# KingOfTheAce2/video-restoration-pipeline-framewright

Measured on AMD Instinct MI355X. Metric: frames/sec Real-ESRGAN x4 1080p (RRDBNet-x4plus, 1920x1080 -> 7680x4320), higher is better.
Workload: dtype f16; 1 GPU; RealESRGAN_x4plus x4, 1920x1080 uint8 BGR frames resident in HBM -> 7680x4320 uint8 BGR in HBM, seeded synthetic weights, 43 frames per GPU

## Files before the change

video-restoration-pipeline-framewright_amd/csrc/conv3x3_wino.hip:

```cpp
#include <cstdlib>
#include <cstring>
#include <type_traits>
#include "fw_internal.h"
#include "conv_common.h"

namespace fw {

constexpr int WN_ROWP = 2 * 17 * 4;
constexpr int WN_ACT = HALO_H * WN_ROWP;
constexpr int WN_ACT_REGION = ACT_INSTR * 64;
constexpr int WN_WFR = 3 * 4 * 4;
constexpr int WN_W_REGION = WN_WFR * 64;
constexpr int WN_TOTAL = WN_ACT_REGION + 2 * WN_W_REGION;
static_assert(NWAVES == 8 && RPW == 2 && WN_TOTAL * 16 <= 160 * 1024, "written for 8 waves of 2 rows");

typedef _Float16 wn_h2 __attribute__((ext_vector_type(2)));
__device__ __forceinline__ uint4 wn_sub(uint4 a, uint4 b) {
    uint4 r;
    r.x = __builtin_bit_cast(unsigned, __builtin_bit_cast(wn_h2, a.x) - __builtin_bit_cast(wn_h2, b.x));
    r.y = __builtin_bit_cast(unsigned, __builtin_bit_cast(wn_h2, a.y) - __builtin_bit_cast(wn_h2, b.y));
    r.z = __builtin_bit_cast(unsigned, __builtin_bit_cast(wn_h2, a.z) - __builtin_bit_cast(wn_h2, b.z));
    r.w = __builtin_bit_cast(unsigned, __builtin_bit_cast(wn_h2, a.w) - __builtin_bit_cast(wn_h2, b.w));
    return r;
}
__device__ __forceinline__ uint4 wn_add(uint4 a, uint4 b) {
    uint4 r;
    r.x = __builtin_bit_cast(unsigned, __builtin_bit_cast(wn_h2, a.x) + __builtin_bit_cast(wn_h2, b.x));
    r.y = __builtin_bit_cast(unsigned, __builtin_bit_cast(wn_h2, a.y) + __builtin_bit_cast(wn_h2, b.y));
    r.z = __builtin_bit_cast(unsigned, __builtin_bit_cast(wn_h2, a.z) + __builtin_bit_cast(wn_h2, b.z));
    r.w = __builtin_bit_cast(unsigned, __builtin_bit_cast(wn_h2, a.w) + __builtin_bit_cast(wn_h2, b.w));
    return r;
}

__device__ __forceinline__ void wn_glds_w6(const void* sbase, unsigned voff, unsigned lds_piece4) {
    const unsigned long long b = (unsigned long long)sbase;
    const unsigned long long sb = ((unsigned long long)(unsigned)__builtin_amdgcn_readfirstlane((unsigned)(b >> 32)) << 32) |
                                  (unsigned long long)(unsigned)__builtin_amdgcn_readfirstlane((unsigned)b);
    lds_piece4 = __builtin_amdgcn_readfirstlane(lds_piece4);
    asm volatile(
        "s_nop 4\n\t"
        "s_mov_b32 m0, %2\n\t"
        "s_nop 0\n\t"
        "global_load_lds_dwordx4 %0, %1 offset:-4096\n\t"
        "global_load_lds_dwordx4 %0, %1 offset:-3072\n\t"
        "global_load_lds_dwordx4 %0, %1 offset:-2048\n\t"
        "global_load_lds_dwordx4 %0, %1 offset:-1024\n\t"
        "global_load_lds_dwordx4 %0, %1\n\t"
        "global_load_lds_dwordx4 %0, %1 offset:1024"
        :
        : "v"(voff), "s"(sb), "s"(lds_piece4)
        : "memory");
}

template <bool PLANES, bool STORE>
__global__ __launch_bounds__(64 * NWAVES, WAVES_PER_SIMD) void conv3x3_wino_split_kernel(const ConvParams p) {
    using T = _Float16;
    __shared__ __attribute__((aligned(16))) uint4 lds[WN_TOTAL];
    const int tid = threadIdx.x;
    const int wave = __builtin_amdgcn_readfirstlane(tid >> 6);
    const int lane = tid & 63;
    const int j = lane & 15;
    const int sl = lane >> 4;

    const int NB = gridDim.x;
    const int xcd = blockIdx.x & 7;
    const int qn = NB >> 3, rn = NB & 7;
    const int lb = (xcd < rn ? xcd * (qn + 1) : rn * (qn + 1) + (xcd - rn) * qn) + (blockIdx.x >> 3);
    const int tiles_x = (p.W + TILE_W - 1) / TILE_W;
    const int tiles_y = (p.H + TILE_H - 1) / TILE_H;
    const int ntiles = tiles_x * tiles_y;
    const int t_lo = (int)((long)lb * ntiles / NB);
    const int t_hi = (int)((long)(lb + 1) * ntiles / NB);
    if (t_lo >= t_hi) return;
    const int nch = p.cin_chunks;
    const int nitems = (t_hi - t_lo) * nch;

    unsigned relb[ACT_ITERS];
    auto piece_pos = [&](int i, int* row, int* px, int* s) {
        int idx = (ACT_ITERS * wave + i) * 64 + lane;
        if (idx >= WN_ACT) idx -= WN_ACT;
        const int rw = idx / WN_ROWP;
        const int rm = idx - rw * WN_ROWP;
        const int par = rm >= 68 ? 1 : 0;
        const int q = rm - 68 * par;
        const int ci = q >> 2;
        *row = rw;
        *px = 2 * ci + par;
        *s = (q & 3) ^ halo_swz(ci);
    };
#pragma unroll
    for (int i = 0; i < ACT_ITERS; ++i) {
        int row, px, s;
        piece_pos(i, &row, &px, &s);
        relb[i] = (unsigned)(((row * p.W + px) * p.in_cstride + s * 8) * 2) + (unsigned)(4 - i) * 1024u;
    }
    const unsigned lds_base = (unsigned)(size_t)(lds_ptr_t)lds;
    const char* in = reinterpret_cast<const char*>(p.in);
    const char* w_b = reinterpret_cast<const char*>(p.wpk);
    const unsigned lane16 = lane * 16;
    const long chunk_bytes = p.in_pstride * 2;

    unsigned a_ok = 0;
    bool a_all = true;
    const char* a_src = nullptr;
    int a_t = t_lo, a_c = 0;
    auto plan_tile = [&]() {
        int aty, atx;
        tile_pos(a_t, tiles_x, tiles_y, &aty, &atx);
        const int ty0 = aty * TILE_H, tx0 = atx * TILE_W;
        a_src = in + ((long)(ty0 - 1) * p.W + (tx0 - 1)) * p.in_cstride * 2;
        a_ok = 0;
#pragma unroll
        for (int i = 0; i < ACT_ITERS; ++i) {
            int row, px, s;
            piece_pos(i, &row, &px, &s);
            const int gy = ty0 - 1 + row, gx = tx0 - 1 + px;
            if ((unsigned)gy < (unsigned)p.H && (unsigned)gx < (unsigned)p.W) a_ok |= 1u << i;
        }
        a_all = __builtin_amdgcn_readfirstlane(__all(a_ok == (1u << ACT_ITERS) - 1u)) != 0;
    };
    auto issue_act = [&]() {
        if (a_c == 0) plan_tile();
        const unsigned dst = (unsigned)(ACT_ITERS * wave * 64);
        if (a_all) {
            glds16_batch_a(a_src, relb, lds_base + (dst + 4 * 64) * 16u);
        } else {
#pragma unroll
            for (int i = 0; i < ACT_ITERS; ++i)
                glds16_v(((a_ok >> i) & 1u) ? a_src + (relb[i] - (unsigned)(4 - i) * 1024u) : reinterpret_cast<const char*>(p.zeros),
                         lds_base + (dst + i * 64) * 16u);
        }
        if (++a_c == nch) {
            a_c = 0;
            ++a_t;
        } else {
            a_src += chunk_bytes;
        }
    };
    auto issue_w = [&](int c, int ws) {
        wn_glds_w6(w_b + (size_t)c * (WN_WFR * 1024) + (6 * wave + 4) * 1024, lane16,
                   lds_base + (unsigned)(WN_ACT_REGION + ws * WN_W_REGION + (6 * wave + 4) * 64) * 16u);
    };

    int rd[4];
#pragma unroll
    for (int k = 0; k < 4; ++k) {
        const int ci = j + (k >> 1);
        rd[k] = (k & 1) * 68 + ci * 4 + (sl ^ halo_swz(ci));
    }
    unsigned id_mask = 0;
#pragma unroll
    for (int ctl = 0; ctl < 2; ++ctl)
#pragma unroll
        for (int e = 0; e < 8; ++e)
            if (16 * ctl + j == 8 * sl + e) id_mask |= 1u << (8 * ctl + e);

    f32x4 acc[RPW][4][4];

    auto add_identity = [&](const uint4 (&xf)[RPW], float sc, int c2, auto freq_tag) {
        constexpr int F = decltype(freq_tag)::value;
#pragma unroll
        for (int ctl = 0; ctl < 2; ++ctl) {
            asm volatile("" : "+v"(sc));
            float e[8];
#pragma unroll
            for (int k = 0; k < 8; ++k) e[k] = ((id_mask >> (8 * ctl + k)) & 1u) ? sc : 0.f;
            const uint2 lo4 = Op<T>::pack4(e[0], e[1], e[2], e[3]);
            const uint2 hi4 = Op<T>::pack4(e[4], e[5], e[6], e[7]);
            const uint4 idf = make_uint4(lo4.x, lo4.y, hi4.x, hi4.y);
#pragma unroll
            for (int row = 0; row < RPW; ++row) {
                if (c2)
                    acc[row][F][2 + ctl] = Op<T>::mfma16(idf, xf[row], acc[row][F][2 + ctl]);
                else
                    acc[row][F][ctl] = Op<T>::mfma16(idf, xf[row], acc[row][F][ctl]);
            }
        }
    };

    auto add_identity1 = [&](int row, const uint4& xf, float sc, int c2, auto freq_tag) {
        constexpr int F = decltype(freq_tag)::value;
#pragma unroll
        for (int ctl = 0; ctl < 2; ++ctl) {
            asm volatile("" : "+v"(sc));
            float e[8];
#pragma unroll
            for (int k = 0; k < 8; ++k) e[k] = ((id_mask >> (8 * ctl + k)) & 1u) ? sc : 0.f;
            const uint2 lo4 = Op<T>::pack4(e[0], e[1], e[2], e[3]);
            const uint2 hi4 = Op<T>::pack4(e[4], e[5], e[6], e[7]);
            const uint4 idf = make_uint4(lo4.x, lo4.y, hi4.x, hi4.y);
            if (c2)
                acc[row][F][2 + ctl] = Op<T>::mfma16(idf, xf, acc[row][F][2 + ctl]);
            else
                acc[row][F][ctl] = Op<T>::mfma16(idf, xf, acc[row][F][ctl]);
        }
    };

    issue_w(0, 0);
    issue_act();

    int n = 0;
    for (int t = t_lo; t < t_hi; ++t) {
        int tty, ttx;
        tile_pos(t, tiles_x, tiles_y, &tty, &ttx);
        const int y0 = tty * TILE_H;
        const int x0 = ttx * TILE_W;
#pragma unroll
        for (int ct = 0; ct < 4; ++ct) {
            const f32x4 bv = *reinterpret_cast<const f32x4*>(p.bias + 16 * ct + 4 * sl);
#pragma unroll
            for (int row = 0; row < RPW; ++row) {
                acc[row][0][ct] = f32x4{0.f, 0.f, 0.f, 0.f};
                acc[row][1][ct] = bv;
                acc[row][2][ct] = f32x4{0.f, 0.f, 0.f, 0.f};
                acc[row][3][ct] = f32x4{0.f, 0.f, 0.f, 0.f};
            }
        }

        for (int c = 0; c < nch; ++c, ++n) {
            if (c > 0 || t == t_lo) FW_WAIT_VMCNT(0);
            __syncthreads();
            uint4 V[4][4];
            const bool own = !STORE && c < 2 && p.in_id_scale != 0.f;
#pragma unroll
            for (int r = 0; r < 4; ++r) {
                const uint4* row = lds + (RPW * wave + r) * WN_ROWP;
                const uint4 d0 = row[rd[0]], d1 = row[rd[1]], d2 = row[rd[2]], d3 = row[rd[3]];
                V[r][0] = wn_sub(d0, d2);
                V[r][1] = wn_add(d1, d2);
                V[r][2] = wn_sub(d2, d1);
                V[r][3] = wn_sub(d1, d3);
                if ((r == 1 || r == 2) && own) {
                    add_identity1(r - 1, d1, p.in_id_scale, c, std::integral_constant<int, 0>{});
                    add_identity1(r - 1, d2, -p.in_id_scale, c, std::integral_constant<int, 3>{});
                }
            }
            __syncthreads();
            const bool more = n + 1 < nitems;
            const int c1 = (c + 1 == nch) ? 0 : c + 1;
#ifndef FW_WN_DMA_K
#define FW_WN_DMA_K -1
#endif
            if (FW_WN_DMA_K < 0 && more) {
                issue_w(c1, (n + 1) & 1);
                issue_act();
            }
            uint4 ix0[RPW], ix1[RPW];
            const bool has_id = PLANES && c < p.n_id;
            const uint4* wl = lds + WN_ACT_REGION + (n & 1) * WN_W_REGION + lane;
#ifndef FW_WN_RING
#define FW_WN_RING 3
#endif
#ifndef FW_WN_RES_K
#define FW_WN_RES_K 17
#endif
            constexpr int RING = FW_WN_RING;
            uint4 wf[RING];
#pragma unroll
            for (int k = 0; k < RING - 1; ++k) wf[k] = wl[k * 64];
            FW_SB();
#pragma unroll
            for (int k = 0; k < WN_WFR; ++k) {
                const int dy = k / 16, f = (k / 4) & 3, ct = k & 3;
                if (k + RING - 1 < WN_WFR) wf[(k + RING - 1) % RING] = wl[(k + RING - 1) * 64];
                FW_SB();
                acc[0][f][ct] = Op<T>::mfma16(wf[k % RING], V[dy][f], acc[0][f][ct]);
                acc[1][f][ct] = Op<T>::mfma16(wf[k % RING], V[dy + 1][f], acc[1][f][ct]);
                FW_SB();
                if (k == FW_WN_DMA_K && more) {
                    issue_w(c1, (n + 1) & 1);
                    issue_act();
                    FW_SB();
                }
                if constexpr (PLANES) {
                    if (k == FW_WN_RES_K) {
                        const char* plane = reinterpret_cast<const char*>(p.in) + p.chunk_off[has_id ? c : 0];
#pragma unroll
                        for (int row = 0; row < RPW; ++row) {
                            const int y = y0 + RPW * wave + row, x = x0 + 2 * j;
                            const int cy = y < p.H ? y : p.H - 1, cx0 = x < p.W ? x : p.W - 1, cx1 = x + 1 < p.W ? x + 1 : p.W - 1;
                            const unsigned rowb = (unsigned)cy * (unsigned)p.W;
                            ix0[row] = *reinterpret_cast<const uint4*>(plane + ((rowb + cx0) * (unsigned)p.in_cstride + 8 * sl) * 2u);
                            ix1[row] = *reinterpret_cast<const uint4*>(plane + ((rowb + cx1) * (unsigned)p.in_cstride + 8 * sl) * 2u);
                        }
                        FW_SB();
                    }
                }
            }
            if constexpr (PLANES) {
                if (has_id) {
#pragma unroll
                    for (int row = 0; row < RPW; ++row) {
                        const int y = y0 + RPW * wave + row, x = x0 + 2 * j;
                        if (!(y < p.H && x < p.W)) ix0[row] = make_uint4(0, 0, 0, 0);
                        if (!(y < p.H && x + 1 < p.W)) ix1[row] = make_uint4(0, 0, 0, 0);
                    }
                    add_identity(ix0, p.id_scale[c], c & 1, std::integral_constant<int, 0>{});
                    add_identity(ix1, -p.id_scale[c], c & 1, std::integral_constant<int, 3>{});
                }
            }
        }

        FW_WAIT_VMCNT(0);
        const int ls = (sl & 1) ? 2 + (sl >> 1) : (sl >> 1);
        const int npass = (!STORE && p.out_lo) ? 2 : 1;
#pragma unroll
        for (int row = 0; row < RPW; ++row) {
            const int y = y0 + RPW * wave + row;
            if (y >= p.H) continue;
#pragma unroll
            for (int ct = 0; ct < 4; ++ct) {
                f32x4 ya = acc[row][0][ct] + acc[row][1][ct] + acc[row][2][ct];
                f32x4 yb = acc[row][1][ct] - acc[row][2][ct] - acc[row][3][ct];
                if constexpr (STORE) {
                    if (p.act == 1) {
                        ya = lrelu4(ya);
                        yb = lrelu4(yb);
                    }
                } else {
                    ya = ya * p.s1;
                    yb = yb * p.s1;
                }
                acc[row][0][ct] = ya;
                acc[row][3][ct] = yb;
            }
            for (int pass = 0; pass < npass; ++pass) {
                char* lane_base = reinterpret_cast<char*>(pass ? p.out_lo : p.out) + ((long)(2 * j) * p.out_cstride + p.out_coff + ls * 8) * 2;
                const long rowoff = ((long)y * p.W + x0) * p.out_cstride * 2;
#pragma unroll
                for (int e = 0; e < 2; ++e)
#pragma unroll
                    for (int c2 = 0; c2 < 2; ++c2) {
                        f32x4 oa = e ? acc[row][3][2 * c2] : acc[row][0][2 * c2], ob = e ? acc[row][3][2 * c2 + 1] : acc[row][0][2 * c2 + 1];
                        if (pass) {
                            oa = oa - Op<T>::unpack4(Op<T>::pack4(oa[0], oa[1], oa[2], oa[3]));
                            ob = ob - Op<T>::unpack4(Op<T>::pack4(ob[0], ob[1], ob[2], ob[3]));
                        }
                        const uint2 pa = Op<T>::pack4(oa[0], oa[1], oa[2], oa[3]);
                        const uint2 pb = Op<T>::pack4(ob[0], ob[1], ob[2], ob[3]);
                        const u32x2 sx = __builtin_amdgcn_permlane16_swap(pa.x, pb.x, false, false);
                        const u32x2 sy = __builtin_amdgcn_permlane16_swap(pa.y, pb.y, false, false);
                        if (x0 + 2 * j + e < p.W)
                            store16(lane_base + rowoff + (long)e * p.out_cstride * 2 + (long)c2 * p.out_pstride * 2, make_uint4(sx[0], sy[0], sx[1], sy[1]));
                    }
            }
        }
    }
}

#undef FW_SB

size_t pack_conv3x3_wino_weights(DType dt, const float* w, int cout, int cin, int cin_chunks, uint16_t* dst) {
    const size_t n = (size_t)cin_chunks * WN_WFR * 64 * 8;
    if (!dst) return n;
    size_t o = 0;
    for (int c = 0; c < cin_chunks; ++c)
        for (int dy = 0; dy < 3; ++dy)
            for (int f = 0; f < 4; ++f)
                for (int ct = 0; ct < 4; ++ct)
                    for (int lane = 0; lane < 64; ++lane)
                        for (int e = 0; e < 8; ++e) {
                            const int co = 16 * ct + (lane & 15), ci = 32 * c + 8 * (lane >> 4) + e;
                            float u = 0.f;
                            if (co < cout && ci < cin) {
                                const float* g = w + ((size_t)co * cin + ci) * 9 + dy * 3;
                                u = f == 0 ? g[0] : f == 1 ? 0.5f * ((g[0] + g[1]) + g[2]) : f == 2 ? 0.5f * ((g[0] - g[1]) + g[2]) : g[2];
                            }
                            dst[o++] = f32_to_operand(dt, u);
                        }
    return n;
}

void check_conv3x3_wino(const ConvParams& p, bool split) {
    if (p.H <= 0 || p.W <= 0 || p.cin_chunks <= 0 || p.upsample2x || !p.out || p.in_cstride < 32 || (p.in_cstride & 7) || (p.out_cstride & 7) ||
        (p.out_coff & 7))
        throw Error(1, "conv3x3_wino: bad problem");
    if (p.in_pstride < 32 || (p.in_pstride & 7) || (p.in_pstride == 32 && p.in_cstride < 32 * p.cin_chunks && (long)p.H * p.W > 1))
        throw Error(1, "conv3x3_wino: bad input channel/plane stride");
    if (p.out_pstride < 32 || (p.out_pstride & 7)) throw Error(1, "conv3x3_wino: bad output plane stride");
    if (p.post_act) throw Error(1, "conv3x3_wino: post_act is not implemented");
    if (p.chan_scale) throw Error(1, "conv3x3_wino: chan_scale is not implemented");
    if (p.res1 || p.res2) throw Error(1, "conv3x3_wino: fp32 residuals (res1 / res2) are not implemented");
    if (p.out_f32) throw Error(1, "conv3x3_wino: the fp32 output copy (out_f32) is not implemented");
    if (p.n_groups > 1) throw Error(1, "conv3x3_wino: output-channel groups (n_groups > 1) are not implemented");
    if (split) {
        if (p.act != 0) throw Error(1, "conv3x3_wino: no activation in the split-trunk form");
        if (p.n_id < 0 || p.n_id > 6 || p.n_id > p.cin_chunks) throw Error(1, "conv3x3_wino: bad number of residual planes (n_id)");
        if (p.n_id > 0 && (long)p.H * p.W * p.in_cstride * 2 > 0xffffffffL) throw Error(1, "conv3x3_wino: residual planes larger than 4 GiB");
        if (operand_to_f32(DT_F16, f32_to_operand(DT_F16, p.in_id_scale)) != p.in_id_scale)
            throw Error(1, "conv3x3_wino: in_id_scale not representable in f16");
        for (int i = 0; i < p.n_id; ++i)
            if (operand_to_f32(DT_F16, f32_to_operand(DT_F16, p.id_scale[i])) != p.id_scale[i])
                throw Error(1, "conv3x3_wino: identity scale not representable in f16");
    } else {
        if (p.act < 0 || p.act > 1) throw Error(1, "conv3x3_wino: act must be 0 or 1 (PReLU is not implemented)");
        if (p.n_id || p.out_lo) throw Error(1, "conv3x3_wino: residual planes / lo planes need the split-trunk form");
    }
}

void launch_conv3x3_wino_split(const ConvParams& p_in, hipStream_t stream) {
    check_conv3x3_wino(p_in, true);
    ConvParams p = p_in;
    p.zeros = conv_zero_page();
    const int tiles = ((p.W + TILE_W - 1) / TILE_W) * ((p.H + TILE_H - 1) / TILE_H);
    const int cus = conv_num_cus();
    dim3 grid(tiles < cus ? tiles : cus), block(64 * NWAVES);
    if (p.n_id > 0)
        hipLaunchKernelGGL((conv3x3_wino_split_kernel<true, false>), grid, block, 0, stream, p);
    else
        hipLaunchKernelGGL((conv3x3_wino_split_kernel<false, false>), grid, block, 0, stream, p);
    FW_HIP_CHECK(hipGetLastError());
}

void launch_conv3x3_wino_store(const ConvParams& p_in, hipStream_t stream) {
    check_conv3x3_wino(p_in, false);
    ConvParams p = p_in;
    p.zeros = conv_zero_page();
    const int tiles = ((p.W + TILE_W - 1) / TILE_W) * ((p.H + TILE_H - 1) / TILE_H);
    const int cus = conv_num_cus();
    dim3 grid(tiles < cus ? tiles : cus), block(64 * NWAVES);
    hipLaunchKernelGGL((conv3x3_wino_split_kernel<false, true>), grid, block, 0, stream, p);
    FW_HIP_CHECK(hipGetLastError());
}

}
```

Baseline: 14.97 frames/s.

## Stream residual planes into per-wave LDS landing zones via global_load_lds

Adds an LZ variant of the split Winograd conv kernel. Instead of loading residual identity planes into registers at a fixed MFMA step, each wave issues direct global-to-LDS DMA loads into its own small landing zone. The residual fragments are spread evenly across input-channel chunks and consumed after a vmcnt wait. The aim is to cut VGPR pressure and spread the residual loads across chunks. In exchange it uses more LDS, adds a full vmcnt wait per chunk that can stall the weight and activation prefetch, and falls back to the old path when the planes exceed 4 GB of addressing or an env var forces it.

Result: no change. 14.97 frames/s, median of 2 (+0.0%).

```diff
diff --git a/video-restoration-pipeline-framewright_amd/csrc/conv3x3_wino.hip b/video-restoration-pipeline-framewright_amd/csrc/conv3x3_wino.hip
--- a/video-restoration-pipeline-framewright_amd/csrc/conv3x3_wino.hip
+++ b/video-restoration-pipeline-framewright_amd/csrc/conv3x3_wino.hip
@@ -12,7 +12,9 @@
 constexpr int WN_WFR = 3 * 4 * 4;
 constexpr int WN_W_REGION = WN_WFR * 64;
 constexpr int WN_TOTAL = WN_ACT_REGION + 2 * WN_W_REGION;
-static_assert(NWAVES == 8 && RPW == 2 && WN_TOTAL * 16 <= 160 * 1024, "written for 8 waves of 2 rows");
+constexpr int WN_ZONE_SLOTS = 3;
+constexpr int WN_ZONE = WN_ZONE_SLOTS * 64;
+static_assert(NWAVES == 8 && RPW == 2 && (WN_TOTAL + NWAVES * WN_ZONE) * 16 <= 160 * 1024, "written for 8 waves of 2 rows");
 
 typedef _Float16 wn_h2 __attribute__((ext_vector_type(2)));
 __device__ __forceinline__ uint4 wn_sub(uint4 a, uint4 b) {
@@ -52,10 +54,54 @@
         : "memory");
 }
 
-template <bool PLANES, bool STORE>
+template <int N>
+__device__ __forceinline__ void wn_glds_res(const char* const (&sbase)[WN_ZONE_SLOTS], const unsigned (&voff)[WN_ZONE_SLOTS], unsigned lds_slot2) {
+    static_assert(N >= 1 && N <= WN_ZONE_SLOTS, "fragments per item");
+    unsigned long long sb[WN_ZONE_SLOTS];
+#pragma unroll
+    for (int i = 0; i < N; ++i) {
+        const unsigned long long b = (unsigned long long)sbase[i];
+        sb[i] = ((unsigned long long)(unsigned)__builtin_amdgcn_readfirstlane((unsigned)(b >> 32)) << 32) |
+                (unsigned long long)(unsigned)__builtin_amdgcn_readfirstlane((unsigned)b);
+    }
+    lds_slot2 = __builtin_amdgcn_readfirstlane(lds_slot2);
+    if constexpr (N == 3)
+        asm volatile(
+            "s_nop 4\n\t"
+            "s_mov_b32 m0, %6\n\t"
+            "s_nop 0\n\t"
+            "global_load_lds_dwordx4 %0, %3 offset:-2048\n\t"
+            "global_load_lds_dwordx4 %1, %4 offset:-1024\n\t"
+            "global_load_lds_dwordx4 %2, %5"
+            :
+            : "v"(voff[0]), "v"(voff[1]), "v"(voff[2]), "s"(sb[0]), "s"(sb[1]), "s"(sb[2]), "s"(lds_slot2)
+            : "memory");
+    else if constexpr (N == 2)
+        asm volatile(
+            "s_nop 4\n\t"
+            "s_mov_b32 m0, %4\n\t"
+            "s_nop 0\n\t"
+            "global_load_lds_dwordx4 %0, %2 offset:-2048\n\t"
+            "global_load_lds_dwordx4 %1, %3 offset:-1024"
+            :
+            : "v"(voff[0]), "v"(voff[1]), "s"(sb[0]), "s"(sb[1]), "s"(lds_slot2)
+            : "memory");
+    else
+        asm volatile(
+            "s_nop 4\n\t"
+            "s_mov_b32 m0, %2\n\t"
+            "s_nop 0\n\t"
+            "global_load_lds_dwordx4 %0, %1 offset:-2048"
+            :
+            : "v"(voff[0]), "s"(sb[0]), "s"(lds_slot2)
+            : "memory");
+}
+
+template <bool PLANES, bool STORE, bool LZ = false>
 __global__ __launch_bounds__(64 * NWAVES, WAVES_PER_SIMD) void conv3x3_wino_split_kernel(const ConvParams p) {
+    static_assert(!LZ || (PLANES && !STORE), "the landing zone is the residual planes'");
     using T = _Float16;
-    __shared__ __attribute__((aligned(16))) uint4 lds[WN_TOTAL];
+    __shared__ __attribute__((aligned(16))) uint4 lds[WN_TOTAL + (LZ ? NWAVES * WN_ZONE : 0)];
     const int tid = threadIdx.x;
     const int wave = __builtin_amdgcn_readfirstlane(tid >> 6);
     const int lane = tid & 63;
@@ -196,6 +242,49 @@
         }
     };
 
+    const int fr_all = 4 * p.n_id;
+    const int fr_q = LZ ? fr_all / nch : 0, fr_r = LZ ? fr_all - fr_q * nch : 0;
+    auto fr_lo = [&](int c) { return c * fr_q + (c < fr_r ? c : fr_r); };
+    const unsigned zone = (unsigned)(WN_TOTAL + wave * WN_ZONE);
+    auto issue_res = [&](int c, int ry0, int rx0) {
+        const int q0 = fr_lo(c), cnt = fr_lo(c + 1) - q0;
+        const char* base[WN_ZONE_SLOTS];
+        unsigned voff[WN_ZONE_SLOTS];
+#pragma unroll
+        for (int s = 0; s < WN_ZONE_SLOTS; ++s) {
+            const int q = q0 + s < fr_all ? q0 + s : fr_all - 1;
+            const int y = ry0 + RPW * wave + ((q >> 1) & 1), x = rx0 + 2 * j + (q & 1);
+            const int cy = y < p.H ? y : p.H - 1, cx = x < p.W ? x : p.W - 1;
+            base[s] = reinterpret_cast<const char*>(p.in) + p.chunk_off[q >> 2];
+            voff[s] = (((unsigned)cy * (unsigned)p.W + (unsigned)cx) * (unsigned)p.in_cstride + 8u * sl) * 2u + (unsigned)(WN_ZONE_SLOTS - 1 - s) * 1024u;
+        }
+        const unsigned dst = lds_base + (zone + (WN_ZONE_SLOTS - 1) * 64) * 16u;
+        if (cnt == 3)
+            wn_glds_res<3>(base, voff, dst);
+        else if (cnt == 2)
+            wn_glds_res<2>(base, voff, dst);
+        else if (cnt == 1)
+            wn_glds_res<1>(base, voff, dst);
+    };
+    auto take_res = [&](int q, int slot, int y0, int x0) {
+        uint4 xf = lds[zone + slot * 64 + lane];
+        const int y = y0 + RPW * wave + ((q >> 1) & 1), x = x0 + 2 * j + (q & 1);
+        if (!(y < p.H && x < p.W)) xf = make_uint4(0, 0, 0, 0);
+        const float sc = p.id_scale[q >> 2];
+        using F0 = std::integral_constant<int, 0>;
+        using F3 = std::integral_constant<int, 3>;
+        switch (q & 7) {
+            case 0: add_identity1(0, xf, sc, 0, F0{}); break;
+            case 1: add_identity1(0, xf, -sc, 0, F3{}); break;
+            case 2: add_identity1(1, xf, sc, 0, F0{}); break;
+            case 3: add_identity1(1, xf, -sc, 0, F3{}); break;
+            case 4: add_identity1(0, xf, sc, 1, F0{}); break;
+            case 5: add_identity1(0, xf, -sc, 1, F3{}); break;
+            case 6: add_identity1(1, xf, sc, 1, F0{}); break;
+            default: add_identity1(1, xf, -sc, 1, F3{}); break;
+        }
+    };
+
     issue_w(0, 0);
     issue_act();
 
@@ -245,6 +334,7 @@
                 issue_w(c1, (n + 1) & 1);
                 issue_act();
             }
+            if constexpr (LZ) issue_res(c, y0, x0);
             uint4 ix0[RPW], ix1[RPW];
             const bool has_id = PLANES && c < p.n_id;
             const uint4* wl = lds + WN_ACT_REGION + (n & 1) * WN_W_REGION + lane;
@@ -272,7 +362,7 @@
                     issue_act();
                     FW_SB();
                 }
-                if constexpr (PLANES) {
+                if constexpr (PLANES && !LZ) {
                     if (k == FW_WN_RES_K) {
                         const char* plane = reinterpret_cast<const char*>(p.in) + p.chunk_off[has_id ? c : 0];
 #pragma unroll
@@ -287,7 +377,16 @@
                     }
                 }
             }
-            if constexpr (PLANES) {
+            if constexpr (LZ) {
+                const int q0 = fr_lo(c), cnt = fr_lo(c + 1) - q0;
+                if (cnt > 0) {
+                    FW_WAIT_VMCNT(0);
+#pragma unroll
+                    for (int s = 0; s < WN_ZONE_SLOTS; ++s)
+                        if (s < cnt) take_res(q0 + s, s, y0, x0);
+                }
+            }
+            if constexpr (PLANES && !LZ) {
                 if (has_id) {
 #pragma unroll
                     for (int row = 0; row < RPW; ++row) {
@@ -405,7 +504,14 @@
     const int tiles = ((p.W + TILE_W - 1) / TILE_W) * ((p.H + TILE_H - 1) / TILE_H);
     const int cus = conv_num_cus();
     dim3 grid(tiles < cus ? tiles : cus), block(64 * NWAVES);
-    if (p.n_id > 0)
+    static const bool force_reg = [] {
+        const char* e = getenv("FW_WINO_PLANES_REG");
+        return e && atoi(e) != 0;
+    }();
+    const bool lz = !force_reg && 4 * p.n_id <= WN_ZONE_SLOTS * p.cin_chunks && (long)p.H * p.W * p.in_cstride * 2 + 2048 <= 0xffffffffL;
+    if (p.n_id > 0 && lz)
+        hipLaunchKernelGGL((conv3x3_wino_split_kernel<true, false, true>), grid, block, 0, stream, p);
+    else if (p.n_id > 0)
         hipLaunchKernelGGL((conv3x3_wino_split_kernel<true, false>), grid, block, 0, stream, p);
     else
         hipLaunchKernelGGL((conv3x3_wino_split_kernel<false, false>), grid, block, 0, stream, p);
```
